# kskjs1203/SevenNet_finetuning

Measured on AMD Instinct MI355X. Metric: atoms/sec energy+force, SevenNet-0 lmax=2, 97,336-atom box @1 GPU, higher is better.
Workload: dtype f32 (MLP / linear products on bf16 MFMA pieces: bf16x6 fwd, bf16x3 bwd); 1 GPU; SevenNet-0 energy+force+virial, 97,336-atom periodic Si box (23^3 cells), 1 GPU; total_atoms=97336, scaling=weak, atoms_per_rank=97336, edges_per_rank=2725408, parallelism=single

## Files before the change

### sevennet_finetuning_amd/csrc/fused.hip

```cpp
#include "cg_tables.h"
#include "common.h"
#include "fused.h"
#include "tp.h"
#include "w2_image.h"

#include <type_traits>


namespace e3gnn {
namespace {

typedef float f32x4 __attribute__((ext_vector_type(4)));

template <int N, int I = 0, class F>
constexpr void sfor_host(F&& f) {
  if constexpr (I < N) {
    f(std::integral_constant<int, I>{});
    sfor_host<N, I + 1>(f);
  }
}
template <int N, int I = 0, class F>
__device__ __forceinline__ void sfor(F&& f) {
  if constexpr (I < N) {
    f(std::integral_constant<int, I>{});
// ... 760 lines not shown
#define E3GNN_DH2_X3 1
#endif
constexpr int LS_PAIR_D = 12288;

__device__ __forceinline__ void dh2_pair_g2(f32x4 (&dh2)[2][4], const float (&dp)[2][4], const float (&dr)[2][4],
                                            bool two, __amdgpu_buffer_rsrc_t w2d, int pair, int lane) {
  bf16x8 d[2][2];
#pragma unroll
  for (int u = 0; u < 2; ++u) {
    float v[8];
#pragma unroll
    for (int t = 0; t < 8; ++t) v[t] = t < 4 ? dp[u][t] : dr[u][t - 4];
    split2x8(v, d[u]);
  }
  bf16x8 a[4][2];
#pragma unroll
  for (int bh = 0; bh < 4; ++bh)
#pragma unroll
    for (int pc = 0; pc < 2; ++pc)
      a[bh][pc] = __builtin_bit_cast(
          bf16x8, __builtin_amdgcn_raw_buffer_load_b128(w2d, lane * 16, pair * LS_PAIR_D + (pc * 4 + bh) * 1024, 0));
#pragma unroll
  for (int bh = 0; bh < 4; ++bh) {
#pragma unroll
    for (int u = 0; u < 2; ++u) {
      if (u == 1 && !two) break;
      dh2[u][bh] = mfma16(a[bh][1], d[u][0], dh2[u][bh]);
      dh2[u][bh] = mfma16(a[bh][0], d[u][1], dh2[u][bh]);
      dh2[u][bh] = mfma16(a[bh][0], d[u][0], dh2[u][bh]);
    }
  }
}

constexpr bool NBR_DH2_BF16 = E3GNN_DH2_X3 != 0;
template <class L>
__global__ __launch_bounds__(256) __attribute__((amdgpu_waves_per_eu(2, 2))) void k_conv_bwd_nbr(
    const int* __restrict__ src_ptr, const int* __restrict__ src_perm, const int* __restrict__ center,
    const float* __restrict__ emb, const float* __restrict__ Y, const float* __restrict__ h,
    const float* __restrict__ gagg, MlpW W, float* __restrict__ dh, float* __restrict__ dgu, int n_centers,
    int r_begin, int r_end, float* __restrict__ demb) {
  __shared__ __attribute__((aligned(16))) float lds[4][L::DX];
  const int wid = threadIdx.x >> 6;
  const int jn = __builtin_amdgcn_readfirstlane(r_begin + blockIdx.x * 4 + wid);
  if (jn >= r_end) return;
  float* dacc = lds[wid];
  const int lane = threadIdx.x & 63, g = lane >> 4, col = lane & 15;
  const int qb = src_ptr[jn], qe = src_ptr[jn + 1];
  const WRes R = make_wres(W, L::W);
  const __amdgpu_buffer_rsrc_t Rx = rsrc_bytes(h + (int64_t)jn * L::DX, L::DX * 4);
  const __amdgpu_buffer_rsrc_t Rg = rsrc_bytes(gagg, (int64_t)n_centers * L::DM * 4);
  for (int t = lane; t < L::DX; t += 64) dacc[t] = 0.f;
  const RowSel rsel = row_scatter_sel(col);
  const int own = row_scatter_own(col);

  for (int q0 = qb; q0 < qe; q0 += 32) {
    const bool two = q0 + 16 < qe;
    phase();
    Op3 wq;
    load_w2b(wq, R.w2b, lane, L::P[0].woff);
    int er[2], vg[2];
    float y[2][9];
    float gu_old[2][3], de_old[2][4];
    Op3 hq[2];
#pragma unroll
    for (int u = 0; u < 2; ++u) {
      const int q = q0 + 16 * u + col;
      er[u] = q < qe ? src_perm[q] : -1;
      vg[u] = (er[u] >= 0 ? center[er[u]] * L::DM : n_centers * L::DM) * 4;
#pragma unroll
      for (int k = 0; k < 9; ++k) y[u][k] = er[u] >= 0 ? Y[(int64_t)er[u] * 9 + k] : 0.f;
#pragma unroll
      for (int k = 0; k < 3; ++k) gu_old[u][k] = (g == 0 && er[u] >= 0) ? dgu[(int64_t)er[u] * 3 + k] : 0.f;
#pragma unroll
      for (int k = 0; k < 4; ++k) de_old[u][k] = (g < 2 && er[u] >= 0) ? demb[(int64_t)er[u] * 8 + 4 * g + k] : 0.f;
      if (u == 1 && !two) continue;
      float b[2];
#pragma unroll
      for (int k = 0; k < 2; ++k) b[k] = er[u] >= 0 ? emb[(int64_t)er[u] * 8 + 4 * k + g] : 0.f;
      MlpT m;
      mlp_chain<CX3>(R, b, lane, m);
      f32x4 h2[4];
#pragma unroll
      for (int bb = 0; bb < 4; ++bb)
#pragma unroll
        for (int r = 0; r < 4; ++r) h2[bb][r] = act_fwd(m.a2[bb][r]);
      split_h2(h2, hq[u]);
    }
    f32x4 dh2[2][4];
#pragma unroll
    for (int u = 0; u < 2; ++u)
#pragma unroll
      for (int bb = 0; bb < 4; ++bb) dh2[u][bb] = zero4();
    float dwp[2][4];
    int nb = 0;
    constexpr int NBLK = L::W / 16;
    f32x4 wcur[2], wnxt[2] = {zero4(), zero4()};
    wcur[0] = w2_block_bwd<false>(hq[0], wq);
    wcur[1] = two ? w2_block_bwd<false>(hq[1], wq) : zero4();
    if (NBLK > 1) load_w2b(wq, R.w2v, lane, 16);
    float dYa[2][9];
#pragma unroll
    for (int u = 0; u < 2; ++u)
#pragma unroll
      for (int k = 0; k < 9; ++k) dYa[u][k] = 0.f;

    sfor<3>([&](auto I) {
      constexpr int MUL = iblock_mul<L, I>();
      if constexpr (MUL > 0) {
        constexpr int D1 = 2 * I + 1;
        constexpr int XOFF = iblock_xoff<L, I>();
        for (int jj = 0; jj < MUL / 16; ++jj) {
          float x[4 * D1], dx[4 * D1];
          phase();
          ldv<4 * D1>(Rx, 4 * g * D1 * 4, (XOFF + 16 * jj * D1) * 4, x);
#pragma unroll
          for (int i = 0; i < 4 * D1; ++i) dx[i] = -0.f;
          sfor<L::NP>([&](auto pi) {
            constexpr PathDef p = L::P[pi];
            if constexpr (p.l1 == I) {
              constexpr int D3 = 2 * p.l3 + 1;
              phase();
              float gm[2][4 * D3];
              load_gm<L, pi>(gm[0], Rg, vg[0], g, jj);
              load_gm<L, pi>(gm[1], Rg, vg[1], g, jj);
              f32x4 bq[4];
              if constexpr (!NBR_DH2_BF16) load_w2q(bq, R.w2r, lane, p.woff + 16 * jj);
              f32x4 wv[2] = {wcur[0], wcur[1]};
              if (nb + 1 < NBLK) {
                wnxt[0] = w2_block_bwd<false>(hq[0], wq);
                wnxt[1] = two ? w2_block_bwd<false>(hq[1], wq) : zero4();
              }
              if (nb + 2 < NBLK) load_w2b(wq, R.w2v, lane, 16 * (nb + 2));
              float dwr2[2][4];
#pragma unroll
              for (int u = 0; u < 2; ++u) {
                if (u == 1 && !two) break;
                float dwr[4];
#pragma unroll
                for (int r = 0; r < 4; ++r) {
                  phase();
                  float dy[2 * p.l2 + 1];
#pragma unroll
                  for (int q = 0; q < 2 * p.l2 + 1; ++q) dy[q] = 0.f;
                  dwr[r] = tp_bwd_xw<p.l1, p.l2, p.l3>(x + r * D1, y[u] + yoff(p.l2), wv[u][r], gm[u] + r * D3,
                                                       dx + r * D1, dy);
                  if constexpr (p.l2 > 0) {
#pragma unroll
                    for (int q = 0; q < 2 * p.l2 + 1; ++q) dYa[u][yoff(p.l2) + q] += dy[q];
                  }
                  pin<D1>(dx + r * D1);
                  pin<8>(dYa[u] + 1);
                }
                if constexpr (NBR_DH2_BF16) {
#pragma unroll
                  for (int r = 0; r < 4; ++r) dwr2[u][r] = u == 1 && !two ? 0.f : dwr[r];
                } else {
#pragma unroll
                  for (int bh = 0; bh < 4; ++bh)
#pragma unroll
                    for (int r = 0; r < 4; ++r) dh2[u][bh] = mfma(bq[bh][r], dwr[r], dh2[u][bh]);
                }
              }
              if constexpr (NBR_DH2_BF16) {
                if (!two) {
#pragma unroll
                  for (int r = 0; r < 4; ++r) dwr2[1][r] = 0.f;
                }
                if (nb & 1) {
                  dh2_pair_g2(dh2, dwp, dwr2, two, R.w2d, nb >> 1, lane);
                } else {
#pragma unroll
                  for (int u = 0; u < 2; ++u)
#pragma unroll
                    for (int r = 0; r < 4; ++r) dwp[u][r] = dwr2[u][r];
                }
              }
              pin<4 * D1>(dx);
              wcur[0] = wnxt[0];
              wcur[1] = wnxt[1];
              ++nb;
            }
          });
          phase();
          {
            constexpr int NV = 4 * D1;
            static_assert(NV % 8 == 4, "batches of 16, 8, then 4");
            float* da = dacc + XOFF + (16 * jj + 4 * g) * D1;
            if constexpr (NV >= 16) da[own] += row_scatter16<16>(dx, rsel);
            if constexpr (NV % 16 >= 8) da[NV / 16 * 16 + (own & 7)] += row_scatter16<8>(dx + NV / 16 * 16, rsel);
            da[NV / 8 * 8 + (own & 3)] += row_scatter16<4>(dx + NV / 8 * 8, rsel);
          }
        }
      }
    });

#pragma unroll
    for (int u = 0; u < 2; ++u) {
      if (u == 1 && !two) break;
      phase();
      float d[8];
#pragma unroll
      for (int q = 0; q < 8; ++q) d[q] = sum_rows4(dYa[u][q + 1]);
      if (g == 0 && er[u] >= 0) {
        const float s3 = 1.7320508075688772f, s5 = 2.23606797749979f, c15 = s3 * s5;
        const float is3 = 0.57735026918962576f;
        const float ux = y[u][1] * is3, uy = y[u][2] * is3, uz = y[u][3] * is3;
        const float gx = s3 * d[0] + c15 * (uz * d[3] + uy * d[4]) - s5 * ux * d[5] - c15 * ux * d[7];
        const float gy = s3 * d[1] + c15 * (ux * d[4] + uz * d[6]) + 2.f * s5 * uy * d[5];
        const float gz = s3 * d[2] + c15 * (ux * d[3] + uy * d[6]) - s5 * uz * d[5] + c15 * uz * d[7];
        float* o = dgu + (int64_t)er[u] * 3;
        o[0] = gu_old[u][0] + gx;
        o[1] = gu_old[u][1] + gy;
        o[2] = gu_old[u][2] + gz;
      }
      phase();
      mlp_bwd_chain_ids(R, emb, er[u], lane, dh2[u], demb, de_old[u]);
    }
  }
  phase();
  __builtin_amdgcn_s_waitcnt(0);
  float* dhj = dh + (int64_t)jn * L::DX;
  for (int t = lane; t < L::DX; t += 64) dhj[t] = dacc[t];
}


constexpr int LS_WPC = E3GNN_BWD_W_X3 ? 2 : 3;
constexpr int LS_DPC = E3GNN_DH2_X3 ? 2 : 3;
constexpr int LS_IMG = (LS_WPC > LS_DPC ? LS_WPC : LS_DPC) * w2img::PIECE_BYTES;

template <int NPC = 3>
__device__ __forceinline__ void lds_op3(Op3& o, const char* pimg, int b, int lane) {
#pragma unroll
  for (int pc = 0; pc < NPC; ++pc)
#pragma unroll
    for (int m = 0; m < 2; ++m) o.v[pc][m] = w2img::tr_read(pimg, lane, b, pc, m);
}

__device__ __forceinline__ void dh2_pair(f32x4 (&dh2)[4], const float (&da)[4], const float (&db)[4],
                                         const char* pimg, int lane) {
  if constexpr (E3GNN_DH2_X3) {
    bf16x8 d[2];
    {
      float v[8];
#pragma unroll
      for (int t = 0; t < 8; ++t) v[t] = t < 4 ? da[t] : db[t - 4];
      split2x8(v, d);
    }
    bf16x8 a[4][2];
#pragma unroll
    for (int bh = 0; bh < 4; ++bh)
#pragma unroll
      for (int pc = 0; pc < 2; ++pc)
        a[bh][pc] = w2img::row_read(pimg, lane, pc, bh);
    phase();
#pragma unroll
    for (int bh = 0; bh < 4; ++bh) {
      dh2[bh] = mfma16(a[bh][1], d[0], dh2[bh]);
      dh2[bh] = mfma16(a[bh][0], d[1], dh2[bh]);
      dh2[bh] = mfma16(a[bh][0], d[0], dh2[bh]);
    }
    return;
  }
  bf16x8 d[3];
  {
    float v[8];
#pragma unroll
    for (int t = 0; t < 8; ++t) v[t] = t < 4 ? da[t] : db[t - 4];
    split3x8(v, d);
  }
  constexpr int I[6] = {2, 1, 0, 1, 0, 0}, J[6] = {0, 1, 2, 0, 1, 0};
#pragma unroll
  for (int bh = 0; bh < 4; ++bh) {
    bf16x8 a[3];
#pragma unroll
    for (int pc = 0; pc < 3; ++pc)
      a[pc] = w2img::row_read(pimg, lane, pc, bh);
#pragma unroll
    for (int q = 0; q < 6; ++q) dh2[bh] = mfma16(a[I[q]], d[J[q]], dh2[bh]);
  }
}

__device__ __forceinline__ int ls_tiles(const int* __restrict__ row_ptr, int cb, int c_end) {
  int T = 0;
#pragma unroll
  for (int w = 0; w < 4; ++w) {
    const int cc = cb + w;
    if (cc < c_end) T = max(T, (row_ptr[cc + 1] - row_ptr[cc] + 15) >> 4);
  }
  return __builtin_amdgcn_readfirstlane(T);
}

template <class L>
struct BwdLsWaves {
  static constexpr int v = L::KIND == 0 ? 3 : 2;
};
constexpr int LS_WPG = 4;
template <class L>
struct LsTwoImages {
  static constexpr int OFF0 = L::KIND == 1 ? L::P[0].mul : 0;
  static constexpr int DMS = L::DM - OFF0;
  static constexpr int bytes = LS_WPG * DMS * 4 + 2 * LS_IMG;
  static constexpr bool v = BwdLsWaves<L>::v * bytes <= 163840;
};
template <int P>
__device__ __forceinline__ void ls_prio() { __builtin_amdgcn_s_setprio(P); }
template <class L>
__global__ __launch_bounds__(64 * LS_WPG) __attribute__((amdgpu_waves_per_eu(BwdLsWaves<L>::v, BwdLsWaves<L>::v))) void k_conv_bwd_ls(
    const int* __restrict__ row_ptr, const int* __restrict__ nbr, const float* __restrict__ emb,
    const float* __restrict__ Y, const float* __restrict__ h, const float* __restrict__ gagg, MlpW W,
    float* __restrict__ dxc, float* __restrict__ dgu, float* __restrict__ demb, int c_begin,
    int c_end, int n_nodes) {
  constexpr int NBLK = L::W / 16, NPAIR = NBLK / 2;
  static_assert(NBLK % 2 == 0, "weight blocks come in pairs");
  constexpr int WPG = LS_WPG, NT = 64 * WPG;
  constexpr int NST = LS_IMG / 16 / NT;
  static_assert(LS_IMG / 16 % NT == 0, "staging pieces per thread");
  constexpr bool TWO = LsTwoImages<L>::v;
  constexpr bool KEEP = BwdLsWaves<L>::v == 2;
  constexpr int OFF0 = TWO ? LsTwoImages<L>::OFF0 : 0, DMS = L::DM - OFF0;
  static_assert(!TWO || (L::P[0].l1 == 0 && L::P[0].l2 == 0 && L::P[0].l3 == 0 && L::P[0].moff == 0 &&
                         OFF0 % 4 == 0), "path 0 is the 0e x 0e -> 0e slice at the row start");
  __shared__ __attribute__((aligned(16))) float smem[WPG * DMS + (TWO ? 2 : 1) * LS_IMG / 4];
  const int tid = threadIdx.x, wid = __builtin_amdgcn_readfirstlane(tid >> 6), lane = tid & 63, g = lane >> 4, col = lane & 15;
  const int cb = c_begin + blockIdx.x * WPG;
  const int c = cb + wid;
  const bool valid = c < c_end;
  const int beg = valid ? row_ptr[c] : 0, end = valid ? row_ptr[c + 1] : 0;
  const int T = ls_tiles(row_ptr, cb, c_end);
  float* dacc = smem + wid * DMS - OFF0;
  char* img = reinterpret_cast<char*>(smem + WPG * DMS);
  if (valid && end > beg) {
    const float4* s4 = reinterpret_cast<const float4*>(gagg + (int64_t)c * L::DM + OFF0);
    float4* d4 = reinterpret_cast<float4*>(dacc + OFF0);
    for (int k = lane; k < DMS / 4; k += 64) d4[k] = s4[k];
  }
  int rb = 0;
  const __amdgpu_buffer_rsrc_t Rg0 =
      rsrc_bytes(gagg + (valid ? (int64_t)c * L::DM : 0), valid ? (int64_t)OFF0 * 4 : 0);
  const WRes R = make_wres(W, L::W);
  const __amdgpu_buffer_rsrc_t Rs = rsrc_bytes(W.w2s, NPAIR * w2img::PAIR_BYTES);
  const __amdgpu_buffer_rsrc_t Rx = rsrc_bytes(h, (int64_t)n_nodes * L::DX * 4);
  f32x4 st[NST];
  auto issue = [&](int P) {
#pragma unroll
    for (int i = 0; i < NST; ++i) st[i] = ldw4(Rs, (tid + NT * i) * 16, P * w2img::PAIR_BYTES);
  };
  auto commit = [&]() {
    __syncthreads();
#pragma unroll
    for (int i = 0; i < NST; ++i) *reinterpret_cast<f32x4*>(img + (tid + NT * i) * 16) = st[i];
    __syncthreads();
  };
  constexpr bool STAMPED = std::is_same<L, LayerMid>::value && !E3GNN_STAMPS_FWD;
  STAMP_DECL
  issue(0);
  for (int t = 0; t < T; ++t) {
    if constexpr (STAMPED) STAMP(0);
    const int q0 = beg + 16 * t;
    const bool act = q0 < end;
    const int er = (act && q0 + col < end) ? q0 + col : -1;
    const int vx = (er >= 0 ? nbr[er] : 0) * L::DX * 4;
    float xpf[20];
    float g0pf[4];
    auto load_group = [&](auto Iq, int jq) {
      constexpr int D1q = 2 * Iq + 1;
      constexpr int XOq = iblock_xoff<L, Iq>();
      ldv<4 * D1q>(Rx, vx + 4 * g * D1q * 4, (XOq + 16 * jq * D1q) * 4, xpf);
      if constexpr (OFF0 > 0 && Iq == 0) ldv<4>(Rg0, 4 * g * 4, 16 * jq * 4, g0pf);
    };
    float y[9];
    float gu_old[3] = {0.f, 0.f, 0.f}, de_old[4] = {0.f, 0.f, 0.f, 0.f};
    f32x4 a2k[4];
    float bk[2];
    Op3 hq;
    load_group(std::integral_constant<int, first_I<L>()>{}, 0);
    const int nrow = (act && dxc) ? min(16, end - q0) : 0;
    const __amdgpu_buffer_rsrc_t Rd =
        rsrc_bytes(dxc ? dxc + (int64_t)(act ? q0 : 0) * L::DX : gagg, (int64_t)nrow * L::DX * 4);
    const int vd = col * L::DX * 4;
    if (act) {
#pragma unroll
      for (int q = 0; q < 9; ++q) y[q] = er >= 0 ? Y[(int64_t)er * 9 + q] : 0.f;
      float b[2];
#pragma unroll
      for (int s = 0; s < 2; ++s) b[s] = er >= 0 ? emb[(int64_t)er * 8 + 4 * s + g] : 0.f;
      if constexpr (KEEP) {
        if (g == 0 && er >= 0) {
#pragma unroll
          for (int k = 0; k < 3; ++k) gu_old[k] = dgu[(int64_t)er * 3 + k];
        }
        if (g < 2 && er >= 0) {
#pragma unroll
          for (int k = 0; k < 4; ++k) de_old[k] = demb[(int64_t)er * 8 + 4 * g + k];
        }
      }
      MlpT m;
      mlp_chain<CX3>(R, b, lane, m);
      if constexpr (KEEP) {
#pragma unroll
        for (int bb = 0; bb < 4; ++bb) a2k[bb] = m.a2[bb];
        bk[0] = b[0];
        bk[1] = b[1];
      }
      f32x4 h2[4];
#pragma unroll
      for (int bb = 0; bb < 4; ++bb)
#pragma unroll
        for (int r = 0; r < 4; ++r) h2[bb][r] = act_fwd(m.a2[bb][r]);
      split_h2(h2, hq);
    }
    if constexpr (STAMPED) STAMP(1);
    f32x4 dh2[4] = {zero4(), zero4(), zero4(), zero4()};
    float dYa[9];
#pragma unroll
    for (int q = 0; q < 9; ++q) dYa[q] = 0.f;
    float dwp[4];
    f32x4 wv0 = zero4(), wv1 = zero4();
    sfor<3>([&](auto I) {
      constexpr int MUL = iblock_mul<L, I>();
      if constexpr (MUL > 0) {
        constexpr int D1 = 2 * I + 1;
        constexpr int XOFF = iblock_xoff<L, I>();
        constexpr int NPI = paths_of<L>(I), U = (NPI & 1) ? 2 : 1, NB0 = blocks_before<L>(I);
        static_assert((MUL / 16) % U == 0, "channel groups come in pairs");
        for (int j2 = 0; j2 < MUL / 16; j2 += U) {
          sfor<U>([&](auto hh) {
            const int jj = j2 + hh;
            float x[4 * D1], dx[4 * D1], g0[4];
#pragma unroll
            for (int i = 0; i < 4 * D1; ++i) {
              x[i] = xpf[i];
              dx[i] = 0.f;
            }
            if constexpr (OFF0 > 0 && I == 0) {
#pragma unroll
              for (int i = 0; i < 4; ++i) g0[i] = g0pf[i];
            }
            if (jj + 1 < MUL / 16) {
              load_group(I, jj + 1);
            } else {
              constexpr int IN = next_I<L>(I);
              if constexpr (IN >= 0) load_group(std::integral_constant<int, IN>{}, 0);
            }
            sfor<L::NP>([&](auto pi) {
              constexpr PathDef p = L::P[pi];
              if constexpr (p.l1 == I) {
                constexpr int D3 = 2 * p.l3 + 1;
                constexpr int ODD = (NB0 + hh * NPI + path_rank<L>(pi)) & 1;
                const int nb = NB0 + jj * NPI + path_rank<L>(pi);
                const char* pimg = img + (TWO ? rb * LS_IMG : 0);
                if constexpr (!ODD) {
                  if constexpr (STAMPED) STAMP(5);
                  const int nextP = (nb >> 1) + 1 < NPAIR ? (nb >> 1) + 1 : 0;
                  if constexpr (TWO) {
#pragma unroll
                    for (int i = 0; i < NST; ++i)
                      *reinterpret_cast<f32x4*>(img + rb * LS_IMG + (tid + NT * i) * 16) = st[i];
                    __syncthreads();
                    issue(nextP);
                  } else {
                    commit();
                    issue(nextP);
                  }
                  if constexpr (STAMPED) STAMP(2);
                  if (act) {
                    ls_prio<1>();
                    Op3 wq, wq1;
                    lds_op3<LS_WPC>(wq, pimg, 0, lane);
                    lds_op3<LS_WPC>(wq1, pimg, 1, lane);
                    phase();
                    wv0 = w2_block_bwd<false>(hq, wq);
                    wv1 = w2_block_bwd<false>(hq, wq1);
                    ls_prio<0>();
                  }
                  if constexpr (STAMPED) STAMP(3);
                }
                if (act) {
                  const f32x4 wv = ODD ? wv1 : wv0;
                  float gm[4 * D3];
                  if constexpr (OFF0 > 0 && pi == 0) {
#pragma unroll
                    for (int k = 0; k < 4; ++k) gm[k] = g0[k];
                  } else {
                    const float* gl = dacc + p.moff + 16 * jj * D3 + 4 * g * D3;
#pragma unroll
                    for (int k = 0; k < 4 * D3; ++k) gm[k] = gl[k];
                  }
                  float dwr[4];
                  tp_bwd_xw4<p.l1, p.l2, p.l3>(x, y + yoff(p.l2), wv, gm, dx, dYa + yoff(p.l2), dwr);
                  if constexpr (L::KIND != 0) pin<4 * D1>(dx);
                  pin<8>(dYa + 1);
                  if constexpr (ODD) {
                    if constexpr (STAMPED) STAMP(5);
                    ls_prio<1>();
                    dh2_pair(dh2, dwp, dwr, pimg, lane);
                    ls_prio<0>();
                    if constexpr (STAMPED) STAMP(4);
                  } else {
#pragma unroll
                    for (int r = 0; r < 4; ++r) dwp[r] = dwr[r];
                  }
                }
                if constexpr (TWO && ODD) rb ^= 1;
              }
            });
            if constexpr (L::KIND != 0)
              stv<4 * D1>(Rd, vd + 4 * g * D1 * 4, (XOFF + 16 * jj * D1) * 4, dx);
          });
        }
      }
    });
    if (act) {
      {
        float d4a[4] = {dYa[1], dYa[2], dYa[3], dYa[4]}, d4b[4] = {dYa[5], dYa[6], dYa[7], dYa[8]};
        sum_rows4_n<4>(d4a);
        sum_rows4_n<4>(d4b);
#pragma unroll
        for (int q = 0; q < 4; ++q) {
          dYa[1 + q] = d4a[q];
          dYa[5 + q] = d4b[q];
        }
      }
      if (g == 0 && er >= 0) {
        const float s3 = 1.7320508075688772f, s5 = 2.23606797749979f, c15 = s3 * s5;
        const float is3 = 0.57735026918962576f;
        const float ux = y[1] * is3, uy = y[2] * is3, uz = y[3] * is3;
        const float* d = dYa + 1;
        const float gx = s3 * d[0] + c15 * (uz * d[3] + uy * d[4]) - s5 * ux * d[5] - c15 * ux * d[7];
        const float gy = s3 * d[1] + c15 * (ux * d[4] + uz * d[6]) + 2.f * s5 * uy * d[5];
        const float gz = s3 * d[2] + c15 * (ux * d[3] + uy * d[6]) - s5 * uz * d[5] + c15 * uz * d[7];
        float* o = dgu + (int64_t)er * 3;
        if constexpr (KEEP) {
          o[0] = gu_old[0] + gx;
          o[1] = gu_old[1] + gy;
          o[2] = gu_old[2] + gz;
        } else {
          o[0] += gx;
          o[1] += gy;
          o[2] += gz;
        }
      }
      if constexpr (STAMPED) STAMP(5);
      mlp_bwd_chain(R, emb, q0, end, lane, dh2, demb, KEEP ? de_old : nullptr, KEEP ? bk : nullptr,
                    KEEP ? a2k : nullptr);
    }
    if constexpr (STAMPED) STAMP(6);
  }
  if constexpr (STAMPED) STAMP_FLUSH(blockIdx.x * WPG + wid);
}

}

template <class L>
static hipError_t bwd_ls_impl(const FusedArgs& a, hipStream_t s) {
  const int nc = a.c_end - a.c_begin;
  hipLaunchKernelGGL(k_conv_bwd_ls<L>, dim3((nc + LS_WPG - 1) / LS_WPG), dim3(64 * LS_WPG), 0, s, a.row_ptr, a.nbr,
                     a.emb, a.Y, a.h, a.gagg, a.W, a.dxc, a.dgu, a.demb, a.c_begin, a.c_end, a.n_nodes);
  return hipGetLastError();
}

template <class L>
static hipError_t fwd_impl(const FusedArgs& a, hipStream_t s) {
  const int nc = a.c_end - a.c_begin;
  if (nc <= 0) return hipSuccess;
  hipLaunchKernelGGL(k_conv_fwd<L>, dim3((nc + 3) / 4), dim3(256), 0, s, a.row_ptr, a.nbr, a.emb,
                     a.Y, a.h, a.agg, a.W, a.c_begin, a.c_end, a.n_nodes, a.denom);
  return hipGetLastError();
}

template <class L>
static hipError_t bwd_nbr_impl(const FusedArgs& a, hipStream_t s) {
  const int nn = a.node_end - a.node_begin;
  hipLaunchKernelGGL(k_conv_bwd_nbr<L>, dim3((nn + 3) / 4), dim3(256), 0, s, a.src_ptr, a.src_perm,
                     a.center, a.emb, a.Y, a.h, a.gagg, a.W, a.dh, a.dgu, a.n_centers, a.node_begin,
                     a.node_end, a.demb);
  return hipGetLastError();
}

#define E3GNN_FAMILY_SWITCH(code, F_FIRST, F_MID, F_LAST)       \
  switch (code) {                                               \
    case 0: F_FIRST(0); case 1: F_MID(0); case 2: F_LAST(0);    \
    case 3: F_FIRST(1); case 4: F_MID(1); case 5: F_LAST(1);    \
    case 6: F_FIRST(2); case 7: F_MID(2); case 8: F_LAST(2);    \
    default: return hipErrorInvalidValue;                       \
  }

hipError_t launch_conv_bwd_ls(int kind, const FusedArgs& a, hipStream_t s) {
  const int nc = a.c_end - a.c_begin;
  if (nc <= 0 || a.n_nodes <= 0) return hipSuccess;
#define FIRST_(f) return bwd_ls_impl<Family<f>::First>(a, s)
#define MID_(f) return bwd_ls_impl<Family<f>::Mid>(a, s)
#define LAST_(f) return hipErrorInvalidValue
  E3GNN_FAMILY_SWITCH(kind, FIRST_, MID_, LAST_)
#undef FIRST_
#undef MID_
#undef LAST_
}

hipError_t launch_conv_fwd(int kind, const FusedArgs& a, hipStream_t s) {
#define FIRST_(f) return fwd_impl<Family<f>::First>(a, s)
#define MID_(f) return fwd_impl<Family<f>::Mid>(a, s)
#define LAST_(f) return fwd_impl<Family<f>::Last>(a, s)
  E3GNN_FAMILY_SWITCH(kind, FIRST_, MID_, LAST_)
#undef FIRST_
#undef MID_
#undef LAST_
}

hipError_t launch_conv_bwd_nbr_last(int kind, const FusedArgs& a, hipStream_t s) {
  const int nn = a.node_end - a.node_begin;
  if (nn <= 0 || a.n_nodes <= 0) return hipSuccess;
#define FIRST_(f) return hipErrorInvalidValue
#define MID_(f) return hipErrorInvalidValue
#define LAST_(f) return bwd_nbr_impl<Family<f>::Last>(a, s)
  E3GNN_FAMILY_SWITCH(kind, FIRST_, MID_, LAST_)
#undef FIRST_
#undef MID_
#undef LAST_
}

template <class L>
static void kind_dims(int* dx, int* w, int* dm) {
  *dx = L::DX;
  *w = L::W;
  *dm = L::DM;
}
bool fused_kind_dims(int code, int* dx, int* w, int* dm) {
  auto f = [&]() -> hipError_t {
#define FIRST_(f) return kind_dims<Family<f>::First>(dx, w, dm), hipSuccess
#define MID_(f) return kind_dims<Family<f>::Mid>(dx, w, dm), hipSuccess
#define LAST_(f) return kind_dims<Family<f>::Last>(dx, w, dm), hipSuccess
    E3GNN_FAMILY_SWITCH(code, FIRST_, MID_, LAST_)
#undef FIRST_
#undef MID_
#undef LAST_
  };
  return f() == hipSuccess;
}

template <class L>
constexpr double kind_tp_flops() {
  double f = 0;
  sfor_host<L::NP>([&](auto pi) {
    constexpr PathDef p = L::P[pi];
    f += (double)p.mul * (2 * CG<p.l1, p.l2, p.l3>::n + 2 * p.l3 + 1);
  });
  return f;
}
static_assert(kind_tp_flops<LayerFirst>() == 3456.0 && kind_tp_flops<LayerMid>() == 16832.0 &&
                  kind_tp_flops<LayerLast>() == 1184.0,
              "SURVEY.md 8d per-edge TP FLOP");
double fused_kind_tp_flops(int code) {
  switch (code) {
#define K_(c, f, T) \
  case c:           \
    return kind_tp_flops<Family<f>::T>();
    K_(0, 0, First) K_(1, 0, Mid) K_(2, 0, Last) K_(3, 1, First) K_(4, 1, Mid) K_(5, 1, Last)
    K_(6, 2, First) K_(7, 2, Mid) K_(8, 2, Last)
#undef K_
    default: return 0.0;
  }
}

template <class L>
static int kind_paths(PathDef* out, int max) {
  for (int p = 0; p < L::NP && p < max; ++p) out[p] = L::P[p];
  return L::NP;
}
int fused_kind_paths(int code, PathDef* out, int max) {
  auto f = [&]() -> int {
    switch (code) {
#define K_(c, f, T) \
  case c:           \
    return kind_paths<Family<f>::T>(out, max);
      K_(0, 0, First) K_(1, 0, Mid) K_(2, 0, Last) K_(3, 1, First) K_(4, 1, Mid) K_(5, 1, Last)
      K_(6, 2, First) K_(7, 2, Mid) K_(8, 2, Last)
#undef K_
      default: return 0;
    }
  };
  return f();
}

}

#ifdef E3GNN_STAMPS
extern "C" int e3gnn_debug_stamps(void* p) {
  return (int)hipMemcpyToSymbol(HIP_SYMBOL(e3gnn::g_stamp_buf), &p, sizeof(p));
}
#endif
```

Baseline: 2.558 million atoms/s.

## Stage two weight pairs per barrier in backward line-sweep conv kernel

For KIND==1 layers where LDS budget and block alignment allow, the backward conv kernel stages two W2 weight-image pairs (four blocks) at once into LDS. This halves the number of __syncthreads/commit points per channel group and lets the prefetch run further ahead. It fully unrolls the channel-group loop at compile time for that case. In exchange it doubles LDS image space and the staging registers, which may raise register pressure and code size.

```diff
diff --git a/sevennet_finetuning_amd/csrc/fused.hip b/sevennet_finetuning_amd/csrc/fused.hip
--- a/sevennet_finetuning_amd/csrc/fused.hip
+++ b/sevennet_finetuning_amd/csrc/fused.hip
@@ -1086,6 +1086,18 @@
   static constexpr int bytes = LS_WPG * DMS * 4 + 2 * LS_IMG;
   static constexpr bool v = BwdLsWaves<L>::v * bytes <= 163840;
 };
+template <class L>
+struct LsQuads {
+  static constexpr int unroll(int npi) { return npi % 4 == 0 ? 1 : npi % 2 == 0 ? 2 : 4; }
+  static constexpr bool pos_ok() {
+    if (L::W / 16 % 4) return false;
+    for (int i = 0; i < 3; ++i)
+      if (mul_of<L>(i) > 0 && (mul_of<L>(i) / 16 % unroll(paths_of<L>(i)) || blocks_before<L>(i) % 4)) return false;
+    return true;
+  }
+  static constexpr int bytes = LS_WPG * (L::DM - LsTwoImages<L>::OFF0) * 4 + 4 * LS_IMG;
+  static constexpr bool v = L::KIND == 1 && LsTwoImages<L>::v && pos_ok() && BwdLsWaves<L>::v * bytes <= 163840;
+};
 template <int P>
 __device__ __forceinline__ void ls_prio() { __builtin_amdgcn_s_setprio(P); }
 template <class L>
@@ -1100,11 +1112,13 @@
   constexpr int NST = LS_IMG / 16 / NT;
   static_assert(LS_IMG / 16 % NT == 0, "staging pieces per thread");
   constexpr bool TWO = LsTwoImages<L>::v;
+  constexpr bool QUAD = LsQuads<L>::v;
+  constexpr int NIMG = QUAD ? 2 : 1;
   constexpr bool KEEP = BwdLsWaves<L>::v == 2;
   constexpr int OFF0 = TWO ? LsTwoImages<L>::OFF0 : 0, DMS = L::DM - OFF0;
   static_assert(!TWO || (L::P[0].l1 == 0 && L::P[0].l2 == 0 && L::P[0].l3 == 0 && L::P[0].moff == 0 &&
                          OFF0 % 4 == 0), "path 0 is the 0e x 0e -> 0e slice at the row start");
-  __shared__ __attribute__((aligned(16))) float smem[WPG * DMS + (TWO ? 2 : 1) * LS_IMG / 4];
+  __shared__ __attribute__((aligned(16))) float smem[WPG * DMS + (TWO ? 2 : 1) * NIMG * LS_IMG / 4];
   const int tid = threadIdx.x, wid = __builtin_amdgcn_readfirstlane(tid >> 6), lane = tid & 63, g = lane >> 4, col = lane & 15;
   const int cb = c_begin + blockIdx.x * WPG;
   const int c = cb + wid;
@@ -1124,10 +1138,11 @@
   const WRes R = make_wres(W, L::W);
   const __amdgpu_buffer_rsrc_t Rs = rsrc_bytes(W.w2s, NPAIR * w2img::PAIR_BYTES);
   const __amdgpu_buffer_rsrc_t Rx = rsrc_bytes(h, (int64_t)n_nodes * L::DX * 4);
-  f32x4 st[NST];
+  f32x4 st[NIMG * NST];
   auto issue = [&](int P) {
 #pragma unroll
-    for (int i = 0; i < NST; ++i) st[i] = ldw4(Rs, (tid + NT * i) * 16, P * w2img::PAIR_BYTES);
+    for (int i = 0; i < NIMG * NST; ++i)
+      st[i] = ldw4(Rs, (tid + NT * (i % NST)) * 16, (P + i / NST) * w2img::PAIR_BYTES);
   };
   auto commit = [&]() {
     __syncthreads();
@@ -1205,9 +1220,10 @@
       if constexpr (MUL > 0) {
         constexpr int D1 = 2 * I + 1;
         constexpr int XOFF = iblock_xoff<L, I>();
-        constexpr int NPI = paths_of<L>(I), U = (NPI & 1) ? 2 : 1, NB0 = blocks_before<L>(I);
+        constexpr int NPI = paths_of<L>(I), NB0 = blocks_before<L>(I);
+        constexpr int U = QUAD ? LsQuads<L>::unroll(NPI) : (NPI & 1) ? 2 : 1;
         static_assert((MUL / 16) % U == 0, "channel groups come in pairs");
-        for (int j2 = 0; j2 < MUL / 16; j2 += U) {
+        auto groups = [&](const int j2) {
           sfor<U>([&](auto hh) {
             const int jj = j2 + hh;
             float x[4 * D1], dx[4 * D1], g0[4];
@@ -1230,16 +1246,16 @@
               constexpr PathDef p = L::P[pi];
               if constexpr (p.l1 == I) {
                 constexpr int D3 = 2 * p.l3 + 1;
-                constexpr int ODD = (NB0 + hh * NPI + path_rank<L>(pi)) & 1;
+                constexpr int POS = (NB0 + hh * NPI + path_rank<L>(pi)) & (2 * NIMG - 1), ODD = POS & 1;
                 const int nb = NB0 + jj * NPI + path_rank<L>(pi);
-                const char* pimg = img + (TWO ? rb * LS_IMG : 0);
-                if constexpr (!ODD) {
+                const char* pimg = img + (TWO ? rb * NIMG * LS_IMG : 0) + (POS >> 1) * LS_IMG;
+                if constexpr (POS == 0) {
                   if constexpr (STAMPED) STAMP(5);
-                  const int nextP = (nb >> 1) + 1 < NPAIR ? (nb >> 1) + 1 : 0;
+                  const int nextP = (nb >> 1) + NIMG < NPAIR ? (nb >> 1) + NIMG : 0;
                   if constexpr (TWO) {
 #pragma unroll
-                    for (int i = 0; i < NST; ++i)
-                      *reinterpret_cast<f32x4*>(img + rb * LS_IMG + (tid + NT * i) * 16) = st[i];
+                    for (int i = 0; i < NIMG * NST; ++i)
+                      *reinterpret_cast<f32x4*>(img + (rb * NIMG + i / NST) * LS_IMG + (tid + NT * (i % NST)) * 16) = st[i];
                     __syncthreads();
                     issue(nextP);
                   } else {
@@ -1247,6 +1263,8 @@
                     issue(nextP);
                   }
                   if constexpr (STAMPED) STAMP(2);
+                }
+                if constexpr (!ODD) {
                   if (act) {
                     ls_prio<1>();
                     Op3 wq, wq1;
@@ -1285,12 +1303,17 @@
                     for (int r = 0; r < 4; ++r) dwp[r] = dwr[r];
                   }
                 }
-                if constexpr (TWO && ODD) rb ^= 1;
+                if constexpr (TWO && POS == 2 * NIMG - 1) rb ^= 1;
               }
             });
             if constexpr (L::KIND != 0)
               stv<4 * D1>(Rd, vd + 4 * g * D1 * 4, (XOFF + 16 * jj * D1) * 4, dx);
           });
+        };
+        if constexpr (QUAD) {
+          sfor<MUL / 16 / U>([&](auto it) { groups(it * U); });
+        } else {
+          for (int j2 = 0; j2 < MUL / 16; j2 += U) groups(j2);
         }
       }
     });
```

After: 2.590 million atoms/s, median of 6. +1.3%, better.
